# matt-suncy/symbols-from-video

Measured on AMD Instinct MI355X. Metric: frames/sec (enc+binarise+dec fwd+bwd), batch 256x256, 1/2/4/8 MI355X, higher is better.
Workload: dtype bf16; 1 GPU; percep_RBVAE fused train step (batch gather from the HBM-resident latent table + fwd+bwd+losses+Adam), item [16,2,8,4,32,32] per GPU = 256 frames/step/GPU (latents of 256x256 frames), latent 32, 4-layer LSTMs, dropout on; parallelism=dp1, graph=True, dist_world_size=1, schedule=one HIP graph per step, devices_visible=1, graphs_captured=1, launcher=torch.distributed.run or self-spawned ranks

## Files before the change

include/rbvae_dbg.h:

```cpp
#ifndef RBVAE_DBG_H
#define RBVAE_DBG_H
#ifdef __cplusplus
extern "C" {
#endif
int rbvae_dbg_mfma_bf16(const void* A, const void* B, float* D, void* stream);
int rbvae_dbg_mfma_f32(const float* A, const float* B, float* D, void* stream);
int rbvae_dbg_glds(const void* src, const int* lane_src_chunk, void* out, void* stream);
int rbvae_dbg_gg_stamps(unsigned long long* buf, void* stream);
int rbvae_dbg_wg_stamps(unsigned long long* buf, void* stream);
int rbvae_dbg_wr_stamps(unsigned long long* buf, void* stream);
int rbvae_dbg_conv_halo_variant(int v);
int rbvae_dbg_lstm_unit_threads(int v);
int rbvae_dbg_tr16(const void* img, const int* rowsel, const int* colsel, void* out, void* stream);

#ifdef __cplusplus
}
#endif
#endif
```

include/rbvae_hip.h:

```cpp
#ifndef RBVAE_HIP_H
#define RBVAE_HIP_H

#include <stddef.h>
#include <stdint.h>

#ifdef __cplusplus
extern "C" {
#endif

#define RBVAE_OK 0
#define RBVAE_E_INVALID (-1)
#define RBVAE_E_LAUNCH (-2)
#define RBVAE_E_UNSUPPORTED (-3)

#define RBVAE_F32 0
#define RBVAE_BF16 1

int rbvae_version(void);
int rbvae_counter_add(unsigned long long* counter, unsigned long long inc, void* stream);
const char* rbvae_last_error(void);

int rbvae_binarize_kl_fwd(const float* h, const float* U, float* y_soft, float* z, float* kl_mean,
                          int rows, int L, float tau, float noise_ratio, float noise_eps, int hard,
                          float kl_p, float kl_eps, int kl_clamp, unsigned long long seed,
// ... 40 lines not shown

size_t rbvae_mse_ws_floats(long n);
int rbvae_mse_fwd(const float* a, const float* b, long n, float* out_mean, float* ws, void* stream);
int rbvae_mse_bwd(const float* a, const float* b, long n, float scale, const float* gscale_dev, float* da,
                  void* stream);

int rbvae_gather_gemm(int dtype, const void* A, const void* W, void* Out, const float* bias, const void* gate,
                      const void* mask, const void* addend, const void* zero_page, int Nimg, int IH, int IW, int TH, int TW, int sa,
                      int OH, int OW, int so, int Kc, int Nout, int lda, int ldo, int taps_total, int nclass,
                      const int* class_desc, int relu, int drop_mode, float drop_p, float scale,
                      unsigned long long seed, const unsigned long long* seed_dev, float* colsum_ws,
                      void* stream);

int rbvae_conv3x3s2_halo_ok(int dtype, int Nimg, int IH, int IW, int Kc, int Nout);
int rbvae_conv3x3s2_halo_colsum_rows(int Nimg, int IH, int IW);
int rbvae_conv3x3s2_halo(int dtype, const void* A, const void* W, void* Out, const float* bias, const void* gate, const void* mask,
                         int Nimg, int IH, int IW, int Kc, int Nout, int lda, int ldo, int relu, int drop_mode, float drop_p,
                         float scale, unsigned long long seed, const unsigned long long* seed_dev, float* colsum_ws, void* stream);

int rbvae_fc_gemm_ok(int dtype, int M, int K, int N, int lda, int ldo);
int rbvae_fc_gemm(int dtype, const void* A, const void* W, void* Out, const float* bias, float* colsum_ws, int M, int K,
                  int N, int lda, int ldo, void* stream);

int rbvae_conv_gather_index(int* idx, int Nimg, int IH, int IW, int OH, int OW, int KH, int KW, int stride,
                            int pad, void* stream);
int rbvae_wgrad_gemm(int dtype, const void* Dy, const void* In, float* dW_slabs, const int* idx,
                     const void* zero_page, int P, int in_rows, int Co, int Ci, int ldy, int ldi, int taps, int ksplit,
                     void* stream);

int rbvae_wgrad3x3s2_halo_ok(int dtype, int Nimg, int OH, int OW, int Ca, int Cb);
int rbvae_wgrad3x3s2_halo_blocks(int Nimg, int OH, int OW);
int rbvae_wgrad3x3s2_halo(int dtype, const void* S, const void* G, float* dW_slabs, const void* zero_page, int Nimg, int OH,
                          int OW, int Ca, int Cb, int lds, int ldg, int ksplit, void* stream);

int rbvae_wgrad3x3s2_row_ok(int dtype, int Nimg, int OH, int OW, int Ca, int Cb);
int rbvae_wgrad3x3s2_row_blocks(int Nimg, int OH, int OW);
int rbvae_wgrad3x3s2_row(int dtype, const void* S, const void* G, float* dW_slabs, const void* zero_page, int Nimg, int OH,
                         int OW, int Ca, int Cb, int lds, int ldg, int ksplit, void* stream);

int rbvae_pack3(int dtype, const float* in, void* out, int d0, int d1, int d2, long s0, long s1, long s2,
                void* stream);
int rbvae_permute_reduce(const float* in, int nslab, long slab_stride, float* out, int d0, int d1, int d2, long s0,
                         long s1, long s2, float scale, int accumulate, void* stream);
int rbvae_cast_pad(int dtype, const float* in, void* out, int rows, int L, int Lpad, void* stream);
int rbvae_reduce_rows(const float* ws, int rows, int C, float* out, float scale, int accumulate, void* stream);
int rbvae_colsum_partial(int dtype, const void* X, int P, int C, int ld, float* ws, void* stream);
size_t rbvae_colsum_ws_floats(int P, int C);
int rbvae_colsum(int dtype, const void* X, int P, int C, int ld, float* out, float* ws, float scale, int accumulate,
                 void* stream);

int rbvae_run_jobs(const void* jobs_dev, int njobs, int blocks_per_job, void* stream);
int rbvae_job_block_map(const long* rows_host, int njobs, int max_blocks_per_job, int* map_host, int map_capacity);
int rbvae_run_jobs_sized(const void* jobs_dev, const void* block_map_dev, int total_blocks, void* stream);

int rbvae_im2col(int dtype, const float* src, long sn, long sc, long sh, long sw, int N, int C, int IH, int IW,
                 int OH, int OW, int KH, int KW, int stride, int pad, int Kpad, void* col, void* stream);
int rbvae_conv_first_fused_ok(int dtype, int Cin, int IH, int IW, int Nout, int N);
int rbvae_conv_first_fused(int dtype, const float* x, int fd1, int fd2, long fs0, long fs1, long fs2, const void* W,
                           const float* bias, const void* zero_page, void* col, void* out, int N, int Cin, int IH, int IW,
                           int Nout, int ldo, int relu, int drop_mode, float drop_p, float scale, unsigned long long seed,
                           const unsigned long long* seed_dev, void* stream);
int rbvae_deconv_last_dgrad_blocks(int dtype, int Cout, int OH, int OW, int C1, int N);
int rbvae_deconv_last_dgrad_fused(int dtype, const float* dpre, const void* W, const void* zero_page, void* col,
                                  const void* gate, void* out, int N, int Cout, int OH, int OW, int C1, int ldo, float scale,
                                  float* colsum_ws, void* stream);

int rbvae_wgrad_first_blocks(int dtype, int Cin, int IH, int IW, int Nout, int N);
int rbvae_wgrad_first(int dtype, int mode, const float* x, int fd1, int fd2, long fs0, long fs1, long fs2, const void* dY,
                      float* dW_slabs, const void* zero_page, int N, int Cin, int IH, int IW, int Nout, int ldy, int ksplit,
                      void* stream);
size_t rbvae_col2im_ws_floats(void);
int rbvae_col2im_nparts(long n_out);
int rbvae_col2im_has_dcol(int N, int IH, int IW, int ldy, int OH, int OW, int Cout);
int rbvae_col2im_sigmoid(int dtype, const void* Y, int ldy, const float* bias, int N, int IH, int IW, int OH,
                         int OW, int Cout, int KH, int KW, int pad, float* xr, const float* target,
                         float* sse_mean, float* ws, float* dpre, float gscale, const float* gscale_dev,
                         void* stream);
int rbvae_im2col_frames(int dtype, const float* src, int fd1, int fd2, long fs0, long fs1, long fs2, long sc, long sh,
                        long sw, int N, int C, int IH, int IW, int OH, int OW, int KH, int KW, int stride, int pad,
                        int Kpad, void* col, void* stream);
int rbvae_col2im_sigmoid_frames(int dtype, const void* Y, int ldy, const float* bias, int N, int IH, int IW, int OH,
                                int OW, int Cout, int KH, int KW, int pad, float* xr, const float* target, int fd1,
                                int fd2, long fs0, long fs1, long fs2, float* sse_mean, float* ws, float* dpre,
                                float gscale, const float* gscale_dev, void* stream);
int rbvae_deconv_last_fused_parts(int dtype, int N, int IH, int IW, int C1, int Cout);
int rbvae_deconv_last_fused(int dtype, const void* D2, const void* V, int NYP, const float* bias, const void* zero_page,
                            int N, int IH, int IW, int C1, int Cout, float* xr, const float* target, int fd1, int fd2,
                            long fs0, long fs1, long fs2, float* ws, float* dpre, float gscale, void* stream);
int rbvae_deconv_last_fwd_bwd_ok(int dtype, int N, int IH, int IW, int C1, int Cout);
int rbvae_deconv_last_fwd_bwd(int dtype, const void* D2, const void* V, int NYP, const void* W, const float* bias,
                              const void* zero_page, int N, int IH, int IW, int C1, int Cout, float* xr, const float* target,
                              int fd1, int fd2, long fs0, long fs1, long fs2, float* ws, float* dpre, float gscale, void* col,
                              void* dd2, float gs, float* colsum_ws, void* stream);
int rbvae_sigmoid_bwd_nhwc(const float* g_nchw, const float* xr_nchw, float* dpre_nhwc, int N, int C, int H, int W,
                           void* stream);
int rbvae_skinny_linear(int dtype, const void* A, const void* B, const float* bias, float* out, int M, int Nc,
                        int K, int lda, int ldb, int ldo, void* stream);
int rbvae_skinny_linear_parts(int dtype, const void* A, const void* B, const float* bias, float* out_parts, int M,
                              int Nc, int K, int lda, int ldb, int ldo, int ksplit, void* stream);

int rbvae_lstm_fwd(const float* wblk, const float* wT, float* hs_all, float* hprev, float* acts, float* cs, int S,
                   int T, int L, int layers, void* stream);
int rbvae_lstm_bwd(const float* wblk, const float* wT, const float* acts, const float* cs, const float* g_top, float* dG,
                   float* dx, int S, int T, int L, int layers, void* stream);
int rbvae_lstm_fwd_wave_ok(int T, int L, int layers);
int rbvae_lstm_bwd_wave_ok(int T, int L, int layers);
// ... 219 lines not shown
```

symbols-from-video_amd/csrc/jobs.hip:

```cpp
#include "common.h"

#ifndef CPK_CIB
#define CPK_CIB 64
#endif
#ifndef JOBS_TILED_ADAM
#define JOBS_TILED_ADAM 1
#endif
#define JOBS_HD __host__ __device__ __forceinline__

namespace rbvae {

enum JobKind : long { JOB_PACK = 0, JOB_PERMUTE, JOB_ROWS, JOB_CONV_PACK, JOB_CONV_REDUCE, JOB_GATHER, JOB_ADAM_PACK, JOB_ADAM };

struct Job {
    long type;
    const float* src;
    void* dst;
    long d0, d1, d2;
    long s0, s1, s2;
    long nslab, slab;
    long dtype;
    long accumulate;
    float scale;
    int fast;
    long inner;
    void* dst2;
    JOBS_HD int type1() const { return (int)(dtype & 255); }
    JOBS_HD int type2() const { return (int)((dtype >> 8) & 255); }
    JOBS_HD long c0() const { return nslab; }
    JOBS_HD long c1() const { return slab; }
    JOBS_HD long c2() const { return accumulate; }
};
static_assert(sizeof(Job) == 16 * 8, "job table stride");


JOBS_HD unsigned job_numel(const Job& j) { return (unsigned)j.d0 * (unsigned)j.d1 * (unsigned)j.d2; }
JOBS_HD unsigned inner_rows_of(const Job& j) { return (unsigned)j.d0 * (unsigned)j.d1; }
JOBS_HD unsigned tail_blocks(const Job& j) {
    if (j.type == JOB_ROWS) return job_numel(j) / 4 + (job_numel(j) % 4 != 0);
    const unsigned n = j.inner ? inner_rows_of(j) : job_numel(j);
    return n / 256 + (n % 256 != 0);
}

JOBS_HD long gather_rows(const Job& j) { return j.d0; }
JOBS_HD long adam_numel(const Job& j) { return j.d0 * j.d1 * j.d2; }
JOBS_HD long adam_flat_blocks(const Job& j) { return (adam_numel(j) + 255) / 256; }

JOBS_HD bool conv_pack_f32(const Job& j) { return j.dtype == RBVAE_F32; }

constexpr int CPK_MAXROW = 2304;
constexpr int CPK_LDS_BYTES = 16 * (CPK_MAXROW + 8);
struct ConvPack {
    unsigned nco, cib, ncb, ngr;
    bool vec_ok;
    JOBS_HD unsigned blocks() const { return ngr * ncb; }
    JOBS_HD unsigned co0(unsigned b) const { return (b / ncb) * nco; }
    JOBS_HD unsigned ci0(unsigned b) const { return (b % ncb) * cib; }
};
JOBS_HD ConvPack conv_pack_geom(const Job& j, unsigned es) {
    const unsigned NCO = 16 / es, NV = 16 / es;
    const unsigned Co = (unsigned)j.d0, Ci = (unsigned)j.d1, kk = (unsigned)j.d2;
    unsigned cib = (CPK_MAXROW / kk) / NV * NV;
    if (cib > Ci) cib = Ci;
    if (cib > CPK_CIB && Ci % CPK_CIB == 0) cib = CPK_CIB;
    const bool vec_ok = (Ci % NV == 0) && (Co % NCO == 0) && ((cib * kk) % 4 == 0) && ((Ci * kk) % 4 == 0);
    return {NCO, cib, (Ci + cib - 1) / cib, (Co + NCO - 1) / NCO, vec_ok};
}

constexpr int CRD_CI = 256, CRD_MAXKK = 16, CRD_ACC = CRD_CI * CRD_MAXKK / 4 / 256;
struct ConvReduce {
    unsigned ncb, nblocks;
    JOBS_HD unsigned blocks() const { return nblocks; }
    JOBS_HD unsigned co(unsigned b) const { return b / ncb; }
    JOBS_HD unsigned ci0(unsigned b) const { return (b % ncb) * CRD_CI; }
};
JOBS_HD ConvReduce conv_reduce_geom(const Job& j) {
    const unsigned ncb = ((unsigned)j.d1 + CRD_CI - 1) / CRD_CI;
    return {ncb, (unsigned)j.d0 * ncb};
}

struct AdamTiles {
    bool tiled;
    int fA, fB;
    unsigned T0, T1, T2, nt0, nt1, nt2;
    JOBS_HD unsigned blocks() const { return nt0 * nt1 * nt2; }
    JOBS_HD unsigned b0(unsigned t) const { return (t / (nt2 * nt1)) * T0; }
    JOBS_HD unsigned b1(unsigned t) const { return ((t / nt2) % nt1) * T1; }
    JOBS_HD unsigned b2(unsigned t) const { return (t % nt2) * T2; }
};
JOBS_HD AdamTiles adam_tiles(const Job& j) {
    AdamTiles g = {};
    if (!(JOBS_TILED_ADAM && j.type == JOB_ADAM_PACK && adam_numel(j) >= (1l << 20))) return g;
    g.fA = j.s0 == 1 ? 0 : (j.s1 == 1 ? 1 : 2);
    g.fB = !j.dst2 ? g.fA : (j.c0() == 1 ? 0 : (j.c1() == 1 ? 1 : 2));
    if (g.fA == 2 && g.fB == 2) return g;
    g.tiled = true;
    const unsigned D0 = (unsigned)j.d0, d1 = (unsigned)j.d1, d2 = (unsigned)j.d2;
    unsigned T0, T1, T2;
    if (g.fA != 2 && g.fB != 2 && g.fA != g.fB) { T2 = 16; T0 = g.fB == 0 ? 32 : 16; T1 = g.fB == 1 ? 32 : 16; }
    else { const int f = g.fA != 2 ? g.fA : g.fB; T2 = 32; T0 = f == 0 ? 32 : 8; T1 = f == 1 ? 32 : 8; }
    g.T0 = T0 < D0 ? T0 : D0; g.T1 = T1 < d1 ? T1 : d1; g.T2 = T2 < d2 ? T2 : d2;
    g.nt0 = (D0 + g.T0 - 1) / g.T0; g.nt1 = (d1 + g.T1 - 1) / g.T1; g.nt2 = (d2 + g.T2 - 1) / g.T2;
    return g;
}

JOBS_HD long job_blocks_of(const Job& j) {
    switch (j.type) {
    case JOB_CONV_PACK: return conv_pack_geom(j, conv_pack_f32(j) ? 4 : 2).blocks();
    case JOB_CONV_REDUCE: return conv_reduce_geom(j).blocks();
    case JOB_GATHER: return gather_rows(j);
    case JOB_ADAM_PACK:
    case JOB_ADAM: { const AdamTiles g = adam_tiles(j); return g.tiled ? (long)g.blocks() : adam_flat_blocks(j); }
    default: return tail_blocks(j);
    }
}

struct AdamCtx {
    float* w; const float* g; float* m; float* v;
    const float* hyper;
    float one_m_b1, b2, one_m_b2, eps, gscale, pad_;
};
static_assert(sizeof(AdamCtx) == 8 * 8, "adam context layout (8 x int64 on the host side)");

__device__ __forceinline__ float adam_value(float w, float g, float& m, float& v, const AdamCtx& c, float step_size,
                                            float bc2_sqrt) {
    return adam_update(w, g, m, v, c.one_m_b1, c.b2, c.one_m_b2, c.eps, c.gscale, step_size, bc2_sqrt);
}
__device__ __forceinline__ float adam_at(const AdamCtx& c, long off, float step_size, float bc2_sqrt) {
    float m = c.m[off], v = c.v[off];
    const float w = adam_value(c.w[off], c.g[off], m, v, c, step_size, bc2_sqrt);
    c.m[off] = m; c.v[off] = v; c.w[off] = w;
    return w;
}

template <typename T>
__device__ __forceinline__ void conv_pack_rows(const Job& j, unsigned char* lds_raw, unsigned bidx, unsigned nblk) {
    constexpr unsigned NCO = 16 / sizeof(T), NV = 16 / sizeof(T);
    typedef __attribute__((ext_vector_type(4))) unsigned u32x4;
    T* tile = (T*)lds_raw;
    const unsigned Co = (unsigned)j.d0, Ci = (unsigned)j.d1, kk = (unsigned)j.d2;
    const ConvPack g = conv_pack_geom(j, sizeof(T));
    const unsigned cib = g.cib;
    const bool vec_ok = g.vec_ok;
    const unsigned pitch = CPK_MAXROW + 8;
    T* wf = (T*)j.dst;
    T* wd = (T*)j.dst2;
    const AdamCtx* actx = (const AdamCtx*)j.inner;
    float step_size = 0.f, bc2_sqrt = 1.f;
    if (actx) { step_size = actx->hyper[0]; bc2_sqrt = actx->hyper[1]; }
    for (unsigned b = bidx; b < g.blocks(); b += nblk) {
        const unsigned co0 = g.co0(b), ci0 = g.ci0(b);
        const unsigned cn = min(cib, Ci - ci0), row = cn * kk;
        __syncthreads();
        if (vec_ok && actx) {
            const unsigned r4 = row / 4, tot = NCO * r4;
            constexpr unsigned AB = 3;
            for (unsigned i0 = threadIdx.x; i0 < tot; i0 += AB * 256) {
                float4 w4[AB], g4[AB], m4[AB], v4[AB];
                long off[AB];
#pragma unroll
                for (unsigned u = 0; u < AB; ++u) {
                    const unsigned i = i0 + u * 256, ic = i < tot ? i : 0;
                    const unsigned r = ic / r4, q = ic - r * r4;
                    off[u] = (j.src - actx->w) + ((long)(co0 + r) * Ci + ci0) * kk + 4 * q;
                    w4[u] = *(const float4*)(actx->w + off[u]); g4[u] = *(const float4*)(actx->g + off[u]);
                    m4[u] = *(const float4*)(actx->m + off[u]); v4[u] = *(const float4*)(actx->v + off[u]);
                }
#pragma unroll
                for (unsigned u = 0; u < AB; ++u) {
                    const unsigned i = i0 + u * 256;
                    if (i < tot) {
                        float4 w = w4[u], m = m4[u], v = v4[u];
                        w.x = adam_value(w.x, g4[u].x, m.x, v.x, *actx, step_size, bc2_sqrt);
                        w.y = adam_value(w.y, g4[u].y, m.y, v.y, *actx, step_size, bc2_sqrt);
                        w.z = adam_value(w.z, g4[u].z, m.z, v.z, *actx, step_size, bc2_sqrt);
                        w.w = adam_value(w.w, g4[u].w, m.w, v.w, *actx, step_size, bc2_sqrt);
                        *(float4*)(actx->w + off[u]) = w; *(float4*)(actx->m + off[u]) = m; *(float4*)(actx->v + off[u]) = v;
                        const unsigned r = i / r4, q = i - r * r4;
                        T* d = tile + r * pitch + 4 * q;
                        Elem<T>::store(d, w.x); Elem<T>::store(d + 1, w.y); Elem<T>::store(d + 2, w.z); Elem<T>::store(d + 3, w.w);
                    }
                }
            }
        } else if (vec_ok) {
            const unsigned r4 = row / 4, tot = NCO * r4;
            constexpr unsigned LB = 9;
            for (unsigned i0 = threadIdx.x; i0 < tot; i0 += LB * 256) {
                float4 v[LB];
#pragma unroll
                for (unsigned u = 0; u < LB; ++u) {
                    const unsigned i = i0 + u * 256, ic = i < tot ? i : 0;
                    const unsigned r = ic / r4, q = ic - r * r4;
                    v[u] = *(const float4*)(j.src + ((size_t)(co0 + r) * Ci + ci0) * kk + 4 * q);
                }
#pragma unroll
                for (unsigned u = 0; u < LB; ++u) {
                    const unsigned i = i0 + u * 256;
// ... 326 lines not shown
#pragma unroll
                for (int i2 = 0; i2 < 16; ++i2) a[i2] += v[i2];
            }
            float* out = (float*)j.dst + lin0;
#pragma unroll
            for (int i2 = 0; i2 < 16; ++i2)
                if ((unsigned)i2 < d2) out[i2] = j.accumulate ? out[i2] + a[i2] * j.scale : a[i2] * j.scale;
        }
    }
}

__device__ __forceinline__ void elem_rows(const Job& j, unsigned bidx, unsigned nblk) {
    const unsigned d0 = (unsigned)j.d0, d1 = (unsigned)j.d1, d2 = (unsigned)j.d2;
    const unsigned n = job_numel(j);
    const int f = j.fast;
    const unsigned ef = f == 0 ? d0 : (f == 1 ? d1 : d2);
    const unsigned em = f == 2 ? d1 : d2;
    for (unsigned i = bidx * 256 + threadIdx.x; i < n; i += nblk * 256) {
        const unsigned fv = i % ef, r = i / ef;
        const unsigned mid = r % em, slow = r / em;
        const unsigned i0 = f == 0 ? fv : slow;
        const unsigned i1 = f == 1 ? fv : (f == 0 ? slow : mid);
        const unsigned i2 = f == 2 ? fv : mid;
        const size_t lin = ((size_t)i0 * d1 + i1) * d2 + i2;
        const size_t so = i0 * (size_t)j.s0 + i1 * (size_t)j.s1 + i2 * (size_t)j.s2;
        if (j.type == JOB_PACK) {
            if (j.dtype == RBVAE_F32) ((float*)j.dst)[so] = j.src[lin];
            else ((bf16_t*)j.dst)[so] = f32_to_bf16(j.src[lin]);
        } else {
            const float* p = j.src + so;
            float a = 0.f;
            const unsigned ns = (unsigned)j.nslab;
            unsigned k = 0;
            for (; k + 16 <= ns; k += 16) {
                float v[16];
#pragma unroll
                for (int u = 0; u < 16; ++u) v[u] = p[(size_t)(k + u) * j.slab];
#pragma unroll
                for (int u = 0; u < 16; ++u) a += v[u];
            }
            for (; k + 4 <= ns; k += 4) {
                const float v0 = p[(size_t)k * j.slab], v1 = p[(size_t)(k + 1) * j.slab];
                const float v2 = p[(size_t)(k + 2) * j.slab], v3 = p[(size_t)(k + 3) * j.slab];
                a = (((a + v0) + v1) + v2) + v3;
            }
            for (; k < ns; ++k) a += p[(size_t)k * j.slab];
            a *= j.scale;
            float* out = (float*)j.dst;
            out[lin] = j.accumulate ? out[lin] + a : a;
        }
    }
}

__global__ __launch_bounds__(256) void run_jobs_k(const Job* __restrict__ jobs, const int4* __restrict__ map) {
    __shared__ __attribute__((aligned(16))) unsigned char lds_raw[CPK_LDS_BYTES];
    static_assert(CPK_LDS_BYTES >= (int)sizeof(float) * CRD_MAXKK * (CRD_CI + 1), "the reduce tile fits the pack tile");
    static_assert(CPK_LDS_BYTES >= 256 * 16, "the wide row reduction's tree fits");
    static_assert(CPK_LDS_BYTES >= (int)sizeof(float) * 32 * 16 * (16 + 1), "the largest Adam tile (adam_tiles) fits");
    unsigned bidx = blockIdx.x, nblk = gridDim.x, jidx = blockIdx.y;
    if (map) {
        const int4 m = map[blockIdx.x];
        jidx = (unsigned)m.x; bidx = (unsigned)m.y; nblk = (unsigned)m.z;
    }
    const Job j = jobs[jidx];
    if (j.type == JOB_CONV_PACK) {
        if (conv_pack_f32(j)) conv_pack_rows<float>(j, lds_raw, bidx, nblk); else conv_pack_rows<bf16_t>(j, lds_raw, bidx, nblk);
        return;
    }
    if (j.type == JOB_CONV_REDUCE) {
        conv_reduce_rows(j, (float*)lds_raw, bidx, nblk);
        return;
    }
    if (j.type == JOB_ADAM_PACK || j.type == JOB_ADAM) {
        adam_rows(j, lds_raw, bidx, nblk);
        return;
    }
    if (j.type == JOB_GATHER) {
        gather_rows_job(j, bidx, nblk);
        return;
    }
    if (bidx >= tail_blocks(j)) return;
    if (j.type == JOB_ROWS) {
        const bool wide = (unsigned)j.nslab >= 1024 && (job_numel(j) & 3) == 0 && ((unsigned)j.slab & 3) == 0 && ((size_t)j.src & 15) == 0;
        if (wide) rows_wide(j, (float4*)lds_raw, bidx, nblk); else rows_wave(j, bidx, nblk);
    } else if (j.inner) {
        inner_rows(j, bidx, nblk);
    } else {
        elem_rows(j, bidx, nblk);
    }
}

}

using namespace rbvae;

extern "C" int rbvae_run_jobs(const void* jobs_dev, int njobs, int blocks_per_job, void* stream) {
    RBVAE_CHECK_ARG(jobs_dev && njobs > 0 && blocks_per_job > 0, "run_jobs: bad arguments");
    RBVAE_CHECK_ARG(njobs <= 65535, "run_jobs: too many jobs");
    hipLaunchKernelGGL(run_jobs_k, dim3(blocks_per_job, njobs), dim3(256), 0, (hipStream_t)stream, (const Job*)jobs_dev,
                       (const int4*)nullptr);
    RBVAE_CHECK_LAUNCH("run_jobs");
    return RBVAE_OK;
}

extern "C" int rbvae_job_block_map(const long* rows_host, int njobs, int max_blocks_per_job, int* map_host, int map_capacity) {
    if (!rows_host || njobs <= 0 || max_blocks_per_job <= 0) return fail(RBVAE_E_INVALID, "job_block_map: bad arguments");
    const Job* jobs = (const Job*)rows_host;
    long total = 0;
    for (int j = 0; j < njobs; ++j) {
        long nb = job_blocks_of(jobs[j]);
        if (nb < 1) nb = 1;
        if (nb > max_blocks_per_job) nb = max_blocks_per_job;
        if (map_host) {
            if (total + nb > map_capacity) return fail(RBVAE_E_INVALID, "job_block_map: map of %d entries is too small", map_capacity);
            for (long b = 0; b < nb; ++b) {
                int* m = map_host + 4 * (total + b);
                m[0] = j; m[1] = (int)b; m[2] = (int)nb; m[3] = 0;
            }
        }
        total += nb;
    }
    if (total >= (1l << 31)) return fail(RBVAE_E_INVALID, "job_block_map: too many workgroups");
    return (int)total;
}

extern "C" int rbvae_run_jobs_sized(const void* jobs_dev, const void* block_map_dev, int total_blocks, void* stream) {
    RBVAE_CHECK_ARG(jobs_dev && block_map_dev && total_blocks > 0, "run_jobs_sized: bad arguments");
    RBVAE_CHECK_ARG((uintptr_t)block_map_dev % 16 == 0, "run_jobs_sized: the block map must be 16-byte aligned");
    hipLaunchKernelGGL(run_jobs_k, dim3(total_blocks), dim3(256), 0, (hipStream_t)stream, (const Job*)jobs_dev,
                       (const int4*)block_map_dev);
    RBVAE_CHECK_LAUNCH("run_jobs_sized");
    return RBVAE_OK;
}
```

symbols-from-video_amd/engine.py:

```python
from __future__ import annotations

import math
import os
from dataclasses import dataclass
from typing import Dict, List, Optional, Sequence, Tuple

import torch

from . import _lib as L
from .jobs import JOB_CONV_PACK, JOB_PACK, JOB_PERMUTE, JOB_ROWS, Col, JobList, JobTable, adam_context
from .jobs import job_block_map

F32, BF16 = 0, 1


@dataclass(frozen=True)
class Variant:
    name: str
    channels: Tuple[int, int, int]
    kernel: int
    lstm_layers: int
    dropout: float
    noise_ratio_arg: bool
    eps: float
# ... 96 lines not shown
class Saved:
    __slots__ = ("N", "S", "T", "hw", "train", "tau", "tau_dev", "hard", "col1", "x_in", "fm_in", "a1", "a2", "a3", "e", "hs_enc", "hp_enc",
                 "acts_enc", "cs_enc", "y", "z", "hs_dec", "hp_dec", "acts_dec", "cs_dec", "ds_pad", "f", "d1", "d2",
                 "xr", "gate_scale", "dpre3", "b3_parts", "dd2_fused")


class Engine:
    def __init__(self, variant: str, in_ch: int, out_ch: int, latent: int, hw: Tuple[int, int],
                 dtype: str = "f32", device: Optional[torch.device] = None):
        if variant not in VARIANTS:
            raise ValueError(f"unknown variant {variant!r}")
        if dtype not in ("f32", "bf16"):
            raise ValueError("dtype must be 'f32' or 'bf16'")
        self.v = VARIANTS[variant]
        self.in_ch, self.out_ch, self.latent = in_ch, out_ch, latent
        self.hw = tuple(hw)
        if self.hw[0] % 8 or self.hw[1] % 8:
            raise ValueError(f"frame size {self.hw} must be divisible by 8 (three stride-2 stages)")
        if latent > 128:
            raise ValueError("latent_dim > 128 is not supported by the LSTM kernel")
        self.dt = F32 if dtype == "f32" else BF16
        self.tdt = torch.float32 if dtype == "f32" else torch.bfloat16
        self.es = 4 if dtype == "f32" else 2
        self.ke = 128 // self.es
        self.layout = ParamLayout(self.v, in_ch, out_ch, latent, self.hw)
        self.device = device or torch.device("cuda", torch.cuda.current_device())
        k = self.v.kernel
        self.k = k
        H, W = self.hw
        self.g1 = (conv_out(H, k), conv_out(W, k))
        self.g2 = (conv_out(self.g1[0], k), conv_out(self.g1[1], k))
        self.g3 = (conv_out(self.g2[0], k), conv_out(self.g2[1], k))
        c1, c2, c3 = self.v.channels
        self.F3 = c3 * self.g3[0] * self.g3[1]
        self.K1 = _ru(k * k * in_ch, self.ke)
        self.K3 = _ru(k * k * out_ch, self.ke)
        self.NY = _ru(k * k * out_ch, 8)
        self.Lp = _ru(latent, self.ke)
        self.zero = torch.zeros(256, dtype=torch.uint8, device=self.device)
        self._cls_conv = conv_classes(k)
        self._cls_dgrad, self._ncls_dgrad = dgrad_classes(k)
        self._desc_cache: Dict[Tuple, object] = {}
        self._idx_cache: Dict[Tuple, torch.Tensor] = {}
        self.seed_dev = None
        self._pack_tab: Dict = {}
        self._bufs: Dict = {}
        self._bwd_tab: Dict = {}
        self._tables: Dict[int, JobTable] = {}
        self._jobs: Optional[JobList] = None
        self._wg_cus = 256
        self.last_wgrad_kernel = None
        self._job_blocks = 256
        self.sized_jobs = 2
        self._side: Optional[torch.cuda.Stream] = None
        self.overlap = True
        self._ks_small = 3
        self.fc_gemm = True
        self.deconv_halo = True
        self._dh_min_wgs = 1024
        self.conv_s2_halo = True
        self._cs_min_wgs = 512
        self._cs_max_waste = 1.15
        self.wgrad_halo = True
        self._wh_min_steps = 8
        self._wh_max_tiles = 2
        self.wgrad_row = True
        self._wr_min_steps = 4
        self._wr_slab_mb = 64
        self._wr_ks_coef = 0.4
        self._wr_min_blocks = 128
        self.wgrad_first = True
        self._wf_min_steps = 8
        self.lstm_pair_bwd = True
        self.keep_dz = False
        ks_unit = 32 if dtype == "bf16" else 16
        wave_ok = latent <= 32 and self.v.lstm_layers * _ru(4 * latent, 64) <= 1024 and not self.v.simple_order
        self.fc_split = 1
        if wave_ok and self.F3 >= 2048:
            for want in ((16, 8, 4) if self.F3 >= 16384 else (4,)):
                if self.F3 % (want * ks_unit) == 0:
                    self.fc_split = want
                    break
        self.lstm_cast = wave_ok
        self.lstm_pair = wave_ok
        self.bin_bwd_fused = wave_ok
        self.deconv_fused = True
        self.conv_first_fused = True
        self.deconv_last_bwd_fused = True
        self._alloc_packed()

    def _alloc_packed(self):
        c1, c2, c3 = self.v.channels
        kk = self.k * self.k
        z = lambda *s: torch.zeros(*s, dtype=self.tdt, device=self.device)
        self.W1p = z(c1, self.K1)
        self.W2f, self.W2d = z(c2, kk, c1), z(c1, kk, c2)
        self.W3f, self.W3d = z(c3, kk, c2), z(c2, kk, c3)
        self.Wfc = z(self.latent, self.F3)
        self.WfcT = z(self.F3, self.Lp)
        self.Wdfc = z(self.F3, self.Lp)
        self.WdfcT = z(self.latent, self.F3)
        self.bdfc = torch.zeros(self.F3, dtype=torch.float32, device=self.device)
        self.V1f, self.V1d = z(c3, kk, c2), z(c2, kk, c3)
        self.V2f, self.V2d = z(c2, kk, c1), z(c1, kk, c2)
        self.V3p = z(self.NY, c1)
        self.V3f = z(c1, self.K3)
        nl, Ld = self.v.lstm_layers, self.latent
        self.wT_enc = torch.zeros(nl, 2, Ld, 4 * Ld, dtype=torch.float32, device=self.device)
        self.wT_dec = torch.zeros(nl, 2, Ld, 4 * Ld, dtype=torch.float32, device=self.device)

    def _upload(self, jl: JobList) -> JobTable:
        t = JobTable(jl, self.device, self._job_blocks)
        self._tables[t.rows.data_ptr()] = t
        return t

    def table_of(self, tab: torch.Tensor) -> Optional[JobTable]:
        return self._tables.get(tab.data_ptr())

    def run_table(self, tab: torch.Tensor, n: int, kind: int = 2):
        t = self._tables.get(tab.data_ptr())
        if t is None or self.sized_jobs < kind:
            L.call("rbvae_run_jobs", tab, n, self._job_blocks)
        else:
            L.call("rbvae_run_jobs_sized", tab, *t.block_map)

    def pack(self, flat: torch.Tensor):
        key = flat.data_ptr()
        t = self._pack_tab.get(key)
        if t is None:
            t = self._pack_tab[key] = self._upload(self._pack_jobs(flat))
        self.run_table(t.rows, t.n)

    def update_jobs(self, flat, gflat, m, v, hyper, betas, eps, gscale, extra_rows=None, part=None):
        key = ("update", flat.data_ptr(), gflat.data_ptr(), m.data_ptr(), v.data_ptr(), hyper.data_ptr(), tuple(betas),
               float(eps), float(gscale), tuple(map(tuple, extra_rows)) if extra_rows else None, part)
        tab = self._pack_tab.get(key)
        if tab is not None:
            return tab.rows, tab.n
        if torch.cuda.is_current_stream_capturing():
            raise RuntimeError("update job table missing during graph capture: run one eager update with the same buffers, "
                               f"hyper-parameters and part ({part!r}) first (FusedTrainer's warm-up steps do)")
        ctx = adam_context(flat, gflat, m, v, hyper, betas, eps, gscale)
        packs_jl = self._pack_jobs(flat)
        by_src: Dict[int, List[List[int]]] = {}
        for row in packs_jl.rows:
            by_src.setdefault(row[Col.SRC], []).append(row)
        lay = self.layout
        jl = JobList()
        jl.rows = [list(r) for r in extra_rows] if extra_rows else []
        jl.keep = [packs_jl.keep]
        o_cut = lay.offsets["decoder_cnn.fc.weight"]
        for name in lay.names:
            src = lay.view(flat, name)
            packs = by_src.pop(src.data_ptr(), [])
            if part is not None and (lay.offsets[name] >= o_cut) != (part == "tail"):
                continue
            kinds = [p_[Col.KIND] for p_ in packs]
            if kinds == [JOB_CONV_PACK]:
                jl.add_conv_pack_adam(packs[0], ctx)
            elif kinds in ([JOB_PACK], [JOB_PACK, JOB_PACK]):
                jl.add_adam_pack(ctx, *packs, what=name)
            elif not packs:
                jl.add_adam(src, ctx)
            else:
                raise RuntimeError(f"{name}: unsupported pack job combination for the fused update")
        if by_src:
            raise RuntimeError("pack jobs whose source is not a parameter tensor")
        tab = self._pack_tab[key] = self._upload(jl)
        return tab.rows, tab.n

    def _pack_jobs(self, flat: torch.Tensor) -> JobList:
        lay, dt = self.layout, self.dt
        c1, c2, c3 = self.v.channels
        kk = self.k * self.k
        g3 = self.g3[0] * self.g3[1]
# ... 683 lines not shown
```

symbols-from-video_amd/jobs.py:

```python
import struct
from enum import IntEnum
from typing import List

import numpy as np
import torch

from . import _lib as L

JOB_PACK, JOB_PERMUTE, JOB_ROWS, JOB_CONV_PACK, JOB_CONV_REDUCE, JOB_GATHER, JOB_ADAM_PACK, JOB_ADAM = range(8)

Col = IntEnum("Col", "KIND SRC DST D0 D1 D2 S0 S1 S2 NSLAB SLAB DTYPE ACCUMULATE SCALE_FAST INNER DST2", start=0)
DIMS, STRIDES = slice(Col.D0, Col.D2 + 1), slice(Col.S0, Col.S2 + 1)


def f32_bits(lo, hi=None):
    if hi is None:
        return struct.unpack("<I", struct.pack("<f", float(lo)))[0]
    return struct.unpack("<q", struct.pack("<ff", float(lo), float(hi)))[0]


def adam_context(flat, gflat, m, v, hyper, betas, eps, gscale):
    b1, b2 = betas
    return torch.tensor([flat.data_ptr(), gflat.data_ptr(), m.data_ptr(), v.data_ptr(), hyper.data_ptr(),
                         f32_bits(1.0 - b1, b2), f32_bits(1.0 - b2, eps), f32_bits(gscale, 0.0)], dtype=torch.int64).to(flat.device)
# ... 28 lines not shown
        assert len(r) == 16, "dims and strides have three entries each"
        return r

    def add_conv_pack(self, src, wf, wd, co, ci, kk, dtype):
        if kk > 16:
            raise ValueError("conv weight pack supports kernels up to 4x4")
        return self._row(JOB_CONV_PACK, [src, wf, wd], (co, ci, kk), SRC=src.data_ptr(), DST=wf.data_ptr(), NSLAB=1, DTYPE=dtype,
                         DST2=wd.data_ptr())

    def add_conv_reduce(self, slabs, dst, co, ci, kk, nslab, scale=1.0):
        return self._row(JOB_CONV_REDUCE, [slabs, dst], (co, ci, kk), SRC=slabs.data_ptr(), DST=dst.data_ptr(), NSLAB=nslab,
                         SLAB=co * kk * ci, SCALE_FAST=f32_bits(scale))

    def add_gather(self, table, out, plan, counter=None):
        keep = [t for t in (table, out, plan, counter) if t is not None]
        return self._row(JOB_GATHER, keep, (plan.shape[1], plan.shape[0], table[0].numel() // 4),
                         SRC=table.data_ptr(), DST=out.data_ptr(), S0=plan.data_ptr(), S1=0 if counter is None else counter.data_ptr(), S2=table.shape[0], NSLAB=1)

    def add_adam(self, src, ctx):
        return self._row(JOB_ADAM, [src, ctx], (src.numel(), 1, 1), SRC=src.data_ptr(), INNER=ctx.data_ptr())

    def add_adam_pack(self, ctx, a, b=None, what="job"):
        if b is None:
            b = [0] * 16
        elif b[DIMS] != a[DIMS]:
            raise RuntimeError(f"{what}: its two packed copies walk different logical shapes")
        r = self._row(JOB_ADAM_PACK, [ctx], a[DIMS], SRC=a[Col.SRC], DST=a[Col.DST], NSLAB=b[Col.S0], SLAB=b[Col.S1],
                      ACCUMULATE=b[Col.S2], DTYPE=a[Col.DTYPE] | (b[Col.DTYPE] << 8), INNER=ctx.data_ptr(), DST2=b[Col.DST])
        r[STRIDES] = a[STRIDES]
        return r

    def add_conv_pack_adam(self, row, ctx):
        return self._row(JOB_CONV_PACK, [ctx], row[DIMS], **{c.name: row[c] for c in (Col.SRC, Col.DST, Col.NSLAB, Col.DTYPE, Col.DST2)},
                         INNER=ctx.data_ptr())

    def upload(self, device):
        return torch.tensor(self.rows, dtype=torch.int64).to(device)

    def signature(self):
        return tuple(tuple(r) for r in self.rows)


def job_block_map(rows, device, cap):
    arr = np.ascontiguousarray(np.array(rows, dtype=np.int64).reshape(len(rows), 16))
    total = L.query("rbvae_job_block_map", arr.ctypes.data, len(rows), cap, None, 0)
    if total <= 0:
        raise RuntimeError("rbvae_job_block_map: " + L.lib().rbvae_last_error().decode())
    m = np.empty(4 * total, dtype=np.int32)
    if L.query("rbvae_job_block_map", arr.ctypes.data, len(rows), cap, m.ctypes.data, total) != total:
        raise RuntimeError("rbvae_job_block_map: " + L.lib().rbvae_last_error().decode())
    return torch.from_numpy(m).to(device), total


class JobTable:

    def __init__(self, jl: JobList, device, cap):
        self.jl, self.n, self.rows = jl, len(jl.rows), jl.upload(device)
        self.block_map = job_block_map(jl.rows, device, cap)
```

Baseline: 591,600 frames/s.

## Size job-kernel LDS dynamically per table and launch heavy blocks first

The job-runner kernel now uses dynamic shared memory sized to the largest job actually in each table, instead of a fixed maximum static allocation, so it can keep more workgroups resident per CU. The conv-pack LDS pitch is shrunk to match the real row length. A host-computed launch order sorts blocks by estimated per-block work, heaviest first, to cut tail imbalance. A debug timestamp path is added but is compiled out by default. The cost is extra host work per launch to recompute LDS size and an extra indirection through the order array.

```diff
diff --git a/include/rbvae_dbg.h b/include/rbvae_dbg.h
--- a/include/rbvae_dbg.h
+++ b/include/rbvae_dbg.h
@@ -9,6 +9,7 @@
 int rbvae_dbg_gg_stamps(unsigned long long* buf, void* stream);
 int rbvae_dbg_wg_stamps(unsigned long long* buf, void* stream);
 int rbvae_dbg_wr_stamps(unsigned long long* buf, void* stream);
+int rbvae_dbg_jobs_stamps(unsigned long long* buf, void* stream);
 int rbvae_dbg_conv_halo_variant(int v);
 int rbvae_dbg_lstm_unit_threads(int v);
 int rbvae_dbg_tr16(const void* img, const int* rowsel, const int* colsel, void* out, void* stream);
diff --git a/include/rbvae_hip.h b/include/rbvae_hip.h
--- a/include/rbvae_hip.h
+++ b/include/rbvae_hip.h
@@ -116,6 +116,10 @@
 int rbvae_run_jobs(const void* jobs_dev, int njobs, int blocks_per_job, void* stream);
 int rbvae_job_block_map(const long* rows_host, int njobs, int max_blocks_per_job, int* map_host, int map_capacity);
 int rbvae_run_jobs_sized(const void* jobs_dev, const void* block_map_dev, int total_blocks, void* stream);
+int rbvae_job_lds_bytes(const long* rows_host, int njobs);
+int rbvae_job_launch_order(const long* rows_host, int njobs, int max_blocks_per_job, int* order_host, int capacity);
+int rbvae_run_jobs_table(const long* rows_host, int njobs, int max_blocks_per_job, const void* jobs_dev,
+                         const void* block_map_dev, const void* order_dev, void* stream);
 
 int rbvae_im2col(int dtype, const float* src, long sn, long sc, long sh, long sw, int N, int C, int IH, int IW,
                  int OH, int OW, int KH, int KW, int stride, int pad, int Kpad, void* col, void* stream);
diff --git a/symbols-from-video_amd/csrc/jobs.hip b/symbols-from-video_amd/csrc/jobs.hip
--- a/symbols-from-video_amd/csrc/jobs.hip
+++ b/symbols-from-video_amd/csrc/jobs.hip
@@ -1,10 +1,15 @@
 #include "common.h"
+#include <algorithm>
+#include <vector>
 
 #ifndef CPK_CIB
 #define CPK_CIB 64
 #endif
 #ifndef JOBS_TILED_ADAM
 #define JOBS_TILED_ADAM 1
+#endif
+#ifndef JOBS_STAMPS
+#define JOBS_STAMPS 0
 #endif
 #define JOBS_HD __host__ __device__ __forceinline__
 
@@ -65,6 +70,11 @@
     if (cib > CPK_CIB && Ci % CPK_CIB == 0) cib = CPK_CIB;
     const bool vec_ok = (Ci % NV == 0) && (Co % NCO == 0) && ((cib * kk) % 4 == 0) && ((Ci * kk) % 4 == 0);
     return {NCO, cib, (Ci + cib - 1) / cib, (Co + NCO - 1) / NCO, vec_ok};
+}
+
+JOBS_HD unsigned conv_pack_pitch(unsigned row, unsigned es) {
+    const unsigned per = 256 / es;
+    return (row + per - 1) / per * per + 8;
 }
 
 constexpr int CRD_CI = 256, CRD_MAXKK = 16, CRD_ACC = CRD_CI * CRD_MAXKK / 4 / 256;
@@ -104,6 +114,30 @@
     return g;
 }
 
+JOBS_HD bool rows_is_wide(const Job& j) {
+    return (unsigned)j.nslab >= 1024 && (job_numel(j) & 3) == 0 && ((unsigned)j.slab & 3) == 0 && ((size_t)j.src & 15) == 0;
+}
+
+JOBS_HD long job_lds_bytes(const Job& j) {
+    switch (j.type) {
+    case JOB_CONV_PACK: {
+        const unsigned es = conv_pack_f32(j) ? 4 : 2, row = conv_pack_geom(j, es).cib * (unsigned)j.d2;
+        return (long)((16 / es - 1) * conv_pack_pitch(row, es) + row) * es;
+    }
+    case JOB_CONV_REDUCE: {
+        const unsigned cn = (unsigned)j.d1 < (unsigned)CRD_CI ? (unsigned)j.d1 : (unsigned)CRD_CI;
+        return (long)(((unsigned)j.d2 - 1) * (cn + 1) + cn) * 4;
+    }
+    case JOB_ADAM_PACK:
+    case JOB_ADAM: {
+        const AdamTiles g = adam_tiles(j);
+        return g.tiled ? (long)((g.T0 * g.T1 - 1) * (g.T2 + 1) + g.T2) * 4 : 0;
+    }
+    case JOB_ROWS: return rows_is_wide(j) ? 256 * 16 : 0;
+    default: return 0;
+    }
+}
+
 JOBS_HD long job_blocks_of(const Job& j) {
     switch (j.type) {
     case JOB_CONV_PACK: return conv_pack_geom(j, conv_pack_f32(j) ? 4 : 2).blocks();
@@ -142,7 +176,7 @@
     const ConvPack g = conv_pack_geom(j, sizeof(T));
     const unsigned cib = g.cib;
     const bool vec_ok = g.vec_ok;
-    const unsigned pitch = CPK_MAXROW + 8;
+    const unsigned pitch = conv_pack_pitch(cib * kk, sizeof(T));
     T* wf = (T*)j.dst;
     T* wd = (T*)j.dst2;
     const AdamCtx* actx = (const AdamCtx*)j.inner;
@@ -575,14 +609,14 @@
     }
 }
 
-__global__ __launch_bounds__(256) void run_jobs_k(const Job* __restrict__ jobs, const int4* __restrict__ map) {
-    __shared__ __attribute__((aligned(16))) unsigned char lds_raw[CPK_LDS_BYTES];
+__device__ __forceinline__ void run_job(const Job* __restrict__ jobs, const int4* __restrict__ map, const int* __restrict__ order,
+                                        unsigned char* lds_raw) {
     static_assert(CPK_LDS_BYTES >= (int)sizeof(float) * CRD_MAXKK * (CRD_CI + 1), "the reduce tile fits the pack tile");
     static_assert(CPK_LDS_BYTES >= 256 * 16, "the wide row reduction's tree fits");
     static_assert(CPK_LDS_BYTES >= (int)sizeof(float) * 32 * 16 * (16 + 1), "the largest Adam tile (adam_tiles) fits");
     unsigned bidx = blockIdx.x, nblk = gridDim.x, jidx = blockIdx.y;
     if (map) {
-        const int4 m = map[blockIdx.x];
+        const int4 m = map[order ? (unsigned)order[blockIdx.x] : blockIdx.x];
         jidx = (unsigned)m.x; bidx = (unsigned)m.y; nblk = (unsigned)m.z;
     }
     const Job j = jobs[jidx];
@@ -604,8 +638,7 @@
     }
     if (bidx >= tail_blocks(j)) return;
     if (j.type == JOB_ROWS) {
-        const bool wide = (unsigned)j.nslab >= 1024 && (job_numel(j) & 3) == 0 && ((unsigned)j.slab & 3) == 0 && ((size_t)j.src & 15) == 0;
-        if (wide) rows_wide(j, (float4*)lds_raw, bidx, nblk); else rows_wave(j, bidx, nblk);
+        if (rows_is_wide(j)) rows_wide(j, (float4*)lds_raw, bidx, nblk); else rows_wave(j, bidx, nblk);
     } else if (j.inner) {
         inner_rows(j, bidx, nblk);
     } else {
@@ -613,15 +646,59 @@
     }
 }
 
+#if JOBS_STAMPS
+constexpr size_t JOBS_STAMP_CAP = 4096, JOBS_STAMP_SLOTS = 16;
+#define JOBS_STAMP_PARAM , unsigned long long* stamps
+#define JOBS_STAMP_ARG , jobs_stamp_slot()
+#define JOBS_STAMP_START const unsigned long long st_t0 = wall_clock64();
+#define JOBS_STAMP_END                                                                                                        \
+    if (stamps) {                                                                                                             \
+        asm volatile("s_waitcnt vmcnt(0)" ::: "memory");                                                                      \
+        __syncthreads();                                                                                                      \
+        if (threadIdx.x == 0 && (size_t)blockIdx.y * gridDim.x + blockIdx.x < JOBS_STAMP_CAP) {                               \
+            unsigned long long* o = stamps + ((size_t)blockIdx.y * gridDim.x + blockIdx.x) * 4;                               \
+            o[0] = st_t0; o[1] = wall_clock64(); o[3] = 0;                                                                    \
+            o[2] = map ? (order ? (unsigned)order[blockIdx.x] : blockIdx.x) : blockIdx.y;                                     \
+        }                                                                                                                     \
+    }
+#else
+#define JOBS_STAMP_PARAM
+#define JOBS_STAMP_ARG
+#define JOBS_STAMP_START
+#define JOBS_STAMP_END
+#endif
+
+__global__ __launch_bounds__(256) void run_jobs_k(const Job* __restrict__ jobs, const int4* __restrict__ map,
+                                                  const int* __restrict__ order JOBS_STAMP_PARAM) {
+    extern __shared__ __attribute__((aligned(16))) unsigned char lds_raw[];
+    JOBS_STAMP_START
+    run_job(jobs, map, order, lds_raw);
+    JOBS_STAMP_END
+}
+
 }
 
 using namespace rbvae;
+
+#if JOBS_STAMPS
+static unsigned long long* g_jobs_stamps = nullptr;
+static unsigned g_jobs_stamp_launch = 0;
+static unsigned long long* jobs_stamp_slot() {
+    return g_jobs_stamps ? g_jobs_stamps + (size_t)(g_jobs_stamp_launch++ % JOBS_STAMP_SLOTS) * JOBS_STAMP_CAP * 4 : nullptr;
+}
+extern "C" int rbvae_dbg_jobs_stamps(unsigned long long* buf, void* stream) {
+    (void)stream;
+    g_jobs_stamps = buf;
+    g_jobs_stamp_launch = 0;
+    return RBVAE_OK;
+}
+#endif
 
 extern "C" int rbvae_run_jobs(const void* jobs_dev, int njobs, int blocks_per_job, void* stream) {
     RBVAE_CHECK_ARG(jobs_dev && njobs > 0 && blocks_per_job > 0, "run_jobs: bad arguments");
     RBVAE_CHECK_ARG(njobs <= 65535, "run_jobs: too many jobs");
-    hipLaunchKernelGGL(run_jobs_k, dim3(blocks_per_job, njobs), dim3(256), 0, (hipStream_t)stream, (const Job*)jobs_dev,
-                       (const int4*)nullptr);
+    hipLaunchKernelGGL(run_jobs_k, dim3(blocks_per_job, njobs), dim3(256), CPK_LDS_BYTES, (hipStream_t)stream, (const Job*)jobs_dev,
+                       (const int4*)nullptr, (const int*)nullptr JOBS_STAMP_ARG);
     RBVAE_CHECK_LAUNCH("run_jobs");
     return RBVAE_OK;
 }
@@ -650,8 +727,84 @@
 extern "C" int rbvae_run_jobs_sized(const void* jobs_dev, const void* block_map_dev, int total_blocks, void* stream) {
     RBVAE_CHECK_ARG(jobs_dev && block_map_dev && total_blocks > 0, "run_jobs_sized: bad arguments");
     RBVAE_CHECK_ARG((uintptr_t)block_map_dev % 16 == 0, "run_jobs_sized: the block map must be 16-byte aligned");
-    hipLaunchKernelGGL(run_jobs_k, dim3(total_blocks), dim3(256), 0, (hipStream_t)stream, (const Job*)jobs_dev,
-                       (const int4*)block_map_dev);
+    hipLaunchKernelGGL(run_jobs_k, dim3(total_blocks), dim3(256), CPK_LDS_BYTES, (hipStream_t)stream, (const Job*)jobs_dev,
+                       (const int4*)block_map_dev, (const int*)nullptr JOBS_STAMP_ARG);
     RBVAE_CHECK_LAUNCH("run_jobs_sized");
     return RBVAE_OK;
 }
+
+static long table_blocks_and_lds(const Job* jobs, int njobs, int max_blocks_per_job, long* lds) {
+    long total = 0, need = 0;
+    for (int j = 0; j < njobs; ++j) {
+        const long nb = job_blocks_of(jobs[j]), l = job_lds_bytes(jobs[j]);
+        total += nb < 1 ? 1 : (nb > max_blocks_per_job ? max_blocks_per_job : nb);
+        if (l > need) need = l;
+    }
+    *lds = (need + 15) / 16 * 16;
+    return total;
+}
+
+extern "C" int rbvae_job_lds_bytes(const long* rows_host, int njobs) {
+    if (!rows_host || njobs <= 0) return fail(RBVAE_E_INVALID, "job_lds_bytes: bad arguments");
+    long lds = 0;
+    table_blocks_and_lds((const Job*)rows_host, njobs, 1, &lds);
+    if (lds > CPK_LDS_BYTES) return fail(RBVAE_E_INVALID, "job_lds_bytes: a job of %ld bytes (at most %d)", lds, CPK_LDS_BYTES);
+    return (int)lds;
+}
+
+static long job_block_weight(const Job& j) {
+    switch (j.type) {
+    case JOB_CONV_PACK: {
+        const long es = conv_pack_f32(j) ? 4 : 2, n = (16 / es) * (long)conv_pack_geom(j, (unsigned)es).cib * j.d2;
+        return n * (4 + 2 * es + (j.inner ? 24 : 0));
+    }
+    case JOB_CONV_REDUCE: return (long)((unsigned)j.d1 < (unsigned)CRD_CI ? j.d1 : CRD_CI) * j.d2 * 4 * (j.nslab + 1);
+    case JOB_GATHER: return j.d2 * 32;
+    case JOB_ADAM_PACK:
+    case JOB_ADAM: {
+        const AdamTiles g = adam_tiles(j);
+        const long n = g.tiled ? (long)g.T0 * g.T1 * g.T2 : (adam_numel(j) < 256 ? adam_numel(j) : 256);
+        return n * (j.type == JOB_ADAM ? 28 : 32);
+    }
+    case JOB_ROWS: return 16 * j.nslab;
+    default: return 256 * 4 * (j.nslab + 1) * (j.inner ? j.d2 : 1);
+    }
+}
+
+extern "C" int rbvae_job_launch_order(const long* rows_host, int njobs, int max_blocks_per_job, int* order_host, int capacity) {
+    if (!rows_host || njobs <= 0 || max_blocks_per_job <= 0 || !order_host) return fail(RBVAE_E_INVALID, "job_launch_order: bad arguments");
+    const Job* jobs = (const Job*)rows_host;
+    long lds = 0;
+    const long total = table_blocks_and_lds(jobs, njobs, max_blocks_per_job, &lds);
+    if (total > capacity) return fail(RBVAE_E_INVALID, "job_launch_order: %ld entries do not fit %d", total, capacity);
+    std::vector<int> by(njobs);
+    std::vector<long> first(njobs), w(njobs);
+    long at = 0;
+    for (int j = 0; j < njobs; ++j) {
+        const long nb = job_blocks_of(jobs[j]);
+        by[j] = j; first[j] = at; w[j] = job_block_weight(jobs[j]);
+        at += nb < 1 ? 1 : (nb > max_blocks_per_job ? max_blocks_per_job : nb);
+    }
+    std::stable_sort(by.begin(), by.end(), [&](int a, int b) { return w[a] > w[b]; });
+    long o = 0;
+    for (int k = 0; k < njobs; ++k) {
+        const int j = by[k];
+        const long end = j + 1 < njobs ? first[j + 1] : total;
+        for (long b = first[j]; b < end; ++b) order_host[o++] = (int)b;
+    }
+    return (int)total;
+}
+
+extern "C" int rbvae_run_jobs_table(const long* rows_host, int njobs, int max_blocks_per_job, const void* jobs_dev,
+                                    const void* block_map_dev, const void* order_dev, void* stream) {
+    RBVAE_CHECK_ARG(rows_host && njobs > 0 && max_blocks_per_job > 0 && jobs_dev && block_map_dev, "run_jobs_table: bad arguments");
+    RBVAE_CHECK_ARG((uintptr_t)block_map_dev % 16 == 0, "run_jobs_table: the block map must be 16-byte aligned");
+    long lds = 0;
+    const long total = table_blocks_and_lds((const Job*)rows_host, njobs, max_blocks_per_job, &lds);
+    RBVAE_CHECK_ARG(total < (1l << 31), "run_jobs_table: too many workgroups");
+    RBVAE_CHECK_ARG(lds <= CPK_LDS_BYTES, "run_jobs_table: a job of %ld bytes of LDS (at most %d)", lds, CPK_LDS_BYTES);
+    hipLaunchKernelGGL(run_jobs_k, dim3((unsigned)total), dim3(256), (size_t)lds, (hipStream_t)stream, (const Job*)jobs_dev,
+                       (const int4*)block_map_dev, (const int*)order_dev JOBS_STAMP_ARG);
+    RBVAE_CHECK_LAUNCH("run_jobs_table");
+    return RBVAE_OK;
+}
diff --git a/symbols-from-video_amd/engine.py b/symbols-from-video_amd/engine.py
--- a/symbols-from-video_amd/engine.py
+++ b/symbols-from-video_amd/engine.py
@@ -172,6 +172,8 @@
         self.last_wgrad_kernel = None
         self._job_blocks = 256
         self.sized_jobs = 2
+        self.table_launch = True
+        self.jobs_heavy_first = 1
         self._side: Optional[torch.cuda.Stream] = None
         self.overlap = True
         self._ks_small = 3
@@ -241,6 +243,8 @@
         t = self._tables.get(tab.data_ptr())
         if t is None or self.sized_jobs < kind:
             L.call("rbvae_run_jobs", tab, n, self._job_blocks)
+        elif self.table_launch:
+            t.run(self.jobs_heavy_first >= kind)
         else:
             L.call("rbvae_run_jobs_sized", tab, *t.block_map)
 
diff --git a/symbols-from-video_amd/jobs.py b/symbols-from-video_amd/jobs.py
--- a/symbols-from-video_amd/jobs.py
+++ b/symbols-from-video_amd/jobs.py
@@ -104,8 +104,32 @@
     return torch.from_numpy(m).to(device), total
 
 
+def job_lds_bytes(rows):
+    arr = np.ascontiguousarray(np.array(rows, dtype=np.int64).reshape(len(rows), 16))
+    n = L.query("rbvae_job_lds_bytes", arr.ctypes.data, len(rows))
+    if n < 0:
+        raise RuntimeError("rbvae_job_lds_bytes: " + L.lib().rbvae_last_error().decode())
+    return n
+
+
+def job_launch_order(rows, cap):
+    arr = np.ascontiguousarray(np.array(rows, dtype=np.int64).reshape(len(rows), 16))
+    total = L.query("rbvae_job_block_map", arr.ctypes.data, len(rows), cap, None, 0)
+    order = np.empty(max(total, 1), dtype=np.int32)
+    if total <= 0 or L.query("rbvae_job_launch_order", arr.ctypes.data, len(rows), cap, order.ctypes.data, total) != total:
+        raise RuntimeError("rbvae_job_launch_order: " + L.lib().rbvae_last_error().decode())
+    return order
+
+
 class JobTable:
 
     def __init__(self, jl: JobList, device, cap):
         self.jl, self.n, self.rows = jl, len(jl.rows), jl.upload(device)
         self.block_map = job_block_map(jl.rows, device, cap)
+        self.cap = cap
+        self.host_rows = np.ascontiguousarray(np.array(jl.rows, dtype=np.int64).reshape(self.n, 16))
+        self.order = torch.from_numpy(job_launch_order(jl.rows, cap)).to(device)
+
+    def run(self, heavy_first=False):
+        L.call("rbvae_run_jobs_table", self.host_rows.ctypes.data, self.n, self.cap, self.rows, self.block_map[0],
+               self.order if heavy_first else None)
```

Result: faster. 600,000 frames/s, median of 6 (+1.4%).
